# zgbkdlm/mfs

Hardware: AMD Instinct MI355X
Metric: filter time-steps/sec (higher is better)
Workload: dtype f64

## Files before the change

include/mfs_hip.h:

```cpp
#ifndef MFS_HIP_H
#define MFS_HIP_H

#include <stdint.h>

#ifdef __cplusplus
extern "C" {
#endif

#define MFS_ABI_VERSION 2

#define MFS_OK 0
#define MFS_EINVAL (-1)
#define MFS_EUNSUPPORTED (-2)
#define MFS_EHIP (-3)
#define MFS_ENOMEM (-4)
#define MFS_ERCCL (-5)

#define MFS_MODE_RAW 0
#define MFS_MODE_CENTRAL 1
#define MFS_MODE_SCALED 2
#define MFS_MODE_ODD_TAIL 0x100

#define MFS_TRANS_OPERATOR 0
#define MFS_TRANS_GAUSSIAN 1
// ... 47 lines not shown
int mfs_pool_trim(int device);
int mfs_pool_stats(int device, uint64_t* device_bytes, uint64_t* pinned_bytes, uint64_t* device_allocs,
                   uint64_t* pinned_allocs);
int mfs_event_create(void** event);
int mfs_event_destroy(void* event);
int mfs_event_record(void* event, void* stream);
int mfs_event_elapsed_ms(void* start, void* stop, float* ms);

int mfs_filter_1d(const mfs_model_1d* model, int mode, int N, int T, int B,
                  const double* m0, int m0_batched, const double* mean0, const double* scale0,
                  const double* ys, int stable,
                  double* out_moments, double* out_means, double* out_scales, double* out_nell,
                  int32_t* out_first_nan, int device, void* stream);

typedef struct mfs_plan_1d mfs_plan_1d;

int mfs_plan_1d_create(mfs_plan_1d** plan, const mfs_model_1d* model , int mode, int N,
                       int T, int B, int stable, int chunk, int device);
int mfs_plan_1d_run(mfs_plan_1d* plan, const double* d_m0, int m0_batched, const double* d_mean0,
                    const double* d_scale0, const double* d_ys, double* d_out_moments, double* d_out_means,
                    double* d_out_scales, double* d_out_nell, int32_t* d_out_first_nan, void* stream);
int mfs_plan_1d_destroy(mfs_plan_1d* plan);
int mfs_plan_1d_geometry(const mfs_plan_1d* plan, int* lanes_per_filter, int* filters_per_block, int* grid,
                         int* lds_bytes_per_block);
#define MFS_BUILD_DENSE 0
#define MFS_BUILD_FAST 1
#define MFS_BUILD_FAST_ONE_WAVE 2
#define MFS_BUILD_FAST_ONE_WAVE_SPEC 3
int mfs_plan_1d_kernel_build(const mfs_plan_1d* plan, int* build);
#define MFS_TRAITS_RUNTIME 0
#define MFS_TRAITS_CENTRAL_TANH_BERNOULLI 1
#define MFS_TRAITS_CENTRAL_IDENTITY_GAUSSIAN 2
int mfs_plan_1d_kernel_traits(const mfs_plan_1d* plan, int* traits);

int mfs_filter_1d_grad(const mfs_model_1d* model, const double* dcoef, const double* dlik, int n_par, int mode, int N,
                       int T, int B, const double* m0, int m0_batched, const double* mean0, const double* scale0,
                       const double* ys, double* out_nell, double* out_grad, int32_t* out_first_nan, int device,
                       void* stream);

int mfs_quadrature_1d(int N, int B, const double* ms, const double* mean, const double* scale, int stable,
                      double* out_weights, double* out_nodes, int device, void* stream);

int mfs_characteristic_1d(int N, int count, const double* ms, const double* mean, const double* scale, int nz,
                          const double* zs, double* out, int device, void* stream);

int mfs_elementary(int which, int n, const double* x, double* out, int device);

#define MFS_ND_TERMS 14
#define MFS_ND_TERMS_MAX 27
#define MFS_ND_ROWS 16
#define MFS_ND_ROWS_MAX 29
#define MFS_ND_TABLE_ROWS(n_terms) ((n_terms) > MFS_ND_TERMS ? MFS_ND_ROWS_MAX : MFS_ND_ROWS)
#define MFS_ND_MAX_EXTENT 6
#define MFS_ND_MAX_EXTENT_HI 7
#define MFS_ND_MAX_FACTORS 2
#define MFS_ND_TRANS_OPERATOR 0
#define MFS_ND_TRANS_GAUSSIAN 1
typedef struct mfs_model_nd {
    int32_t d;
    int32_t trans_kind;
    int32_t n_terms;
    int32_t extent;
    int32_t n_factors;
    int32_t ny;
    int32_t fac_kind[MFS_ND_MAX_FACTORS];
    int32_t fac_component[MFS_ND_MAX_FACTORS];
// ... 131 lines not shown
```

mfs_amd/_lib.py:

```python
import ctypes as C
import os

import numpy as np

_HERE = os.path.dirname(os.path.abspath(__file__))
LIB_PATH = os.path.join(_HERE, 'libmfs_hip.so')

MFS_OK = 0
MODE = {'raw': 0, 'central': 1, 'scaled': 2}
MODE_ODD_TAIL = 0x100
TRANS = {'operator': 0, 'gaussian': 1}
UMAP = {'x': 0, 'tanh': 1}
LIK = {'bernoulli_logistic': 0, 'poisson_softplus': 1, 'gaussian': 2, 'bearing_gaussian': 3}
MAX_N = 32
GRID_MAX_N = 8192
PF_MAX_PARTICLES = 1 << 20
PF_MAX_MIX = 8
RESAMPLE = {'stratified': 0, 'systematic': 1}
GF_METHOD = {'sigma_point': 0, 'ekf': 1}
GF_MAX_POINTS = 256

c_double_p = C.POINTER(C.c_double)
c_int32_p = C.POINTER(C.c_int32)

# ... 62 lines not shown
    ('mfs_version', _i, []),
    ('mfs_last_error', C.c_char_p, []),
    ('mfs_device_count', _i, [C.POINTER(C.c_int)]),
    ('mfs_set_device', _i, [_i]),
    ('mfs_device_synchronize', _i, []),
    ('mfs_device_name', _i, [_i, C.c_char_p, _i]),
    ('mfs_malloc', _i, [_vpp, _u64]),
    ('mfs_free', _i, [_vp]),
    ('mfs_memcpy_h2d', _i, [_vp, _vp, _u64, _vp]),
    ('mfs_memcpy_d2h', _i, [_vp, _vp, _u64, _vp]),
    ('mfs_memset', _i, [_vp, _i, _u64, _vp]),
    ('mfs_host_alloc', _i, [_vpp, _u64, _i]),
    ('mfs_host_free', _i, [_vp]),
    ('mfs_pool_trim', _i, [_i]),
    ('mfs_pool_stats', _i, [_i, C.POINTER(_u64), C.POINTER(_u64), C.POINTER(_u64), C.POINTER(_u64)]),
    ('mfs_stream_create', _i, [_vpp]),
    ('mfs_stream_destroy', _i, [_vp]),
    ('mfs_stream_synchronize', _i, [_vp]),
    ('mfs_event_create', _i, [_vpp]),
    ('mfs_event_destroy', _i, [_vp]),
    ('mfs_event_record', _i, [_vp, _vp]),
    ('mfs_event_elapsed_ms', _i, [_vp, _vp, C.POINTER(C.c_float)]),
    ('mfs_filter_1d', _i, [C.POINTER(MfsModel1d), _i, _i, _i, _i, _vp, _i, _vp, _vp, _vp, _i,
                           _vp, _vp, _vp, _vp, _vp, _i, _vp]),
    ('mfs_filter_1d_grad', _i, [C.POINTER(MfsModel1d), _vp, _vp, _i, _i, _i, _i, _i, _vp, _i, _vp, _vp, _vp, _vp, _vp, _vp,
                                _i, _vp]),
    ('mfs_plan_1d_create', _i, [_vpp, C.POINTER(MfsModel1d), _i, _i, _i, _i, _i, _i, _i]),
    ('mfs_plan_1d_run', _i, [_vp, _vp, _i, _vp, _vp, _vp, _vp, _vp, _vp, _vp, _vp, _vp]),
    ('mfs_plan_1d_destroy', _i, [_vp]),
    ('mfs_plan_1d_geometry', _i, [_vp, C.POINTER(C.c_int), C.POINTER(C.c_int), C.POINTER(C.c_int),
                                  C.POINTER(C.c_int)]),
    ('mfs_plan_1d_kernel_build', _i, [_vp, C.POINTER(C.c_int)]),
    ('mfs_plan_1d_kernel_traits', _i, [_vp, C.POINTER(C.c_int)]),
    ('mfs_quadrature_1d', _i, [_i, _i, _vp, _vp, _vp, _i, _vp, _vp, _i, _vp]),
    ('mfs_characteristic_1d', _i, [_i, _i, _vp, _vp, _vp, _i, _vp, _vp, _i, _vp]),
    ('mfs_filter_nd', _i, [C.POINTER(MfsModelNd), _i, _i, _i, _i, _i, _vp, _vp, _vp, _i, _vp, _vp, _vp, _i,
                           _vp, _vp, _vp, _vp, _vp, _i, _vp]),
    ('mfs_plan_nd_create', _i, [_vpp, C.POINTER(MfsModelNd), _i, _i, _i, _i, _i, _vp, _vp, _i, _i]),
    ('mfs_plan_nd_run', _i, [_vp, _vp, _i, _vp, _vp, _vp, _vp, _vp, _vp, _vp, _vp, _vp]),
    ('mfs_plan_nd_destroy', _i, [_vp]),
    ('mfs_plan_nd_geometry', _i, [_vp, C.POINTER(C.c_int), C.POINTER(C.c_int), C.POINTER(C.c_int)]),
    ('mfs_filter_nd3', _i, [C.POINTER(MfsModelNd3), _i, _i, _i, _i, _i, _vp, _vp, _vp, _i, _vp, _vp, _vp, _i,
                            _vp, _vp, _vp, _vp, _vp, _i, _vp]),
    ('mfs_plan_nd3_create', _i, [_vpp, C.POINTER(MfsModelNd3), _i, _i, _i, _i, _i, _vp, _vp, _i, _i]),
    ('mfs_plan_nd3_run', _i, [_vp, _vp, _i, _vp, _vp, _vp, _vp, _vp, _vp, _vp, _vp, _vp]),
    ('mfs_plan_nd3_destroy', _i, [_vp]),
    ('mfs_plan_nd3_geometry', _i, [_vp, C.POINTER(C.c_int), C.POINTER(C.c_int), C.POINTER(C.c_int)]),
    ('mfs_filter_nd3_joint', _i, [C.POINTER(MfsModelNd3), C.POINTER(MfsJointNd3), _i, _i, _i, _i, _i, _vp, _vp, _vp, _i, _vp,
                                  _vp, _vp, _i, _vp, _vp, _vp, _vp, _vp, _i, _vp]),
    ('mfs_plan_nd3_create_joint', _i, [_vpp, C.POINTER(MfsModelNd3), C.POINTER(MfsJointNd3), _i, _i, _i, _i, _i, _vp, _vp, _i,
                                       _i]),
    ('mfs_elementary', _i, [_i, _i, _vp, _vp, _i]),
    ('mfs_grid_filter_1d', _i, [_i, _i, _i, _i, _i, _vp, _vp, _vp, _i, _i, _vp, _i, _vp, _i, _vp,
                                _vp, _vp, _vp, _vp, _vp, _i, _vp]),
    ('mfs_grid_gemm_dev', _i, [_i, _i, _i, _vp, _vp, _vp, _vp]),
    ('mfs_particle_filter_1d', _i, [C.POINTER(MfsModel1d), _i, _i, _i, _i, _vp, _i, _vp, _vp, _vp, _vp, _i, _vp, _i, _vp,
                                    _vp, _vp, _vp, _vp, _vp, _vp, _i, _vp]),
    ('mfs_pf_draws', _i, [_u64, _i, _i, _i, _i, _vp, _vp, _i]),
    ('mfs_pf_last_split_ms', _i, [_vp]),
    ('mfs_gaussian_filter_1d', _i, [C.POINTER(MfsModel1d), _i, _i, _vp, _vp, _i, _i, _vp, _vp, _i, _vp, _vp, _vp, _vp, _vp,
                                    _i, _vp]),
    ('mfs_gaussian_filter_nd', _i, [C.POINTER(MfsModelNd), _i, _i, _vp, _vp, _i, _i, _vp, _vp, _i, _vp, _vp, _vp, _vp, _vp,
                                    _i, _vp]),
    ('mfs_comm_unique_id', _i, [_vp]),
    ('mfs_comm_init', _i, [_vpp, _vp, _i, _i, _i]),
    ('mfs_allgather_nell', _i, [_vp, _vp, _vp, _u64, _vp]),
# ... 137 lines not shown
```

mfs_amd/csrc/capi.hip:

```cpp
#include <hip/hip_runtime.h>

#include <cmath>
#include <cstdarg>
#include <cstdio>
#include <cstdlib>
#include <cstring>
#include <dlfcn.h>
#include <mutex>
#include <string>
#include <vector>

#include "filternd_kernel.hpp"
#include "filternd3_kernel.hpp"
#include "filter1d_grad.hpp"
#include "registry.hpp"
#include "staging.hpp"

namespace mfs {
KernelEntry g_table[MFS_MAX_N + 1][kSlots];
FastEntry g_fast[MFS_MAX_N + 1][4];

thread_local std::string g_err;

int fail(int code, const char* fmt, ...) {
// ... 46 lines not shown
    if (const char* e = getenv("MFS_LANES_PER_FILTER")) want = atoi(e);
    if ((stable != 0 || odd_tail != 0) && want != 0) dense = true;
    if (dense) {
        int gi = (N <= 16) ? 0 : (N <= 32) ? 1 : 2;
        if (want == 64) gi = 2;
        else if (want == 32 && N <= 32) gi = 1;
        else if (want == 16 && N <= 16) gi = 0;
        return gi;
    }
    int gi = mfs::default_group(N);
    if (want == 64) gi = 2;
    else if (want == 32 && N + 1 <= 32) gi = 1;
    else if (want == 16 && N + 1 <= 16) gi = 0;
    else if (want == 8 && N + 1 <= 8) gi = 3;
    return 3 + gi;
}

int check_run_pointers(int mode, const double* m0, const double* mean0, const double* scale0, const double* ys,
                       const double* out_nell, int T, int B) {
    if (!m0 || !out_nell || (T > 0 && B > 0 && !ys)) return fail(MFS_EINVAL, "m0 / ys / out_nell must not be NULL");
    if (mode != MFS_MODE_RAW && !mean0) return fail(MFS_EINVAL, "mean0 is required in central and scaled modes");
    if (mode == MFS_MODE_SCALED && !scale0) return fail(MFS_EINVAL, "scale0 is required in scaled mode");
    return MFS_OK;
}

}

struct mfs_plan_1d {
    mfs_model_1d model;
    int mode, N, T, B, stable, chunk, device, extra;
    int G, fpb, grid, lds_bytes, lds_doubles;
    mfs::Filter1dLaunch launch = nullptr;
    int launch_lds = 0, build = MFS_BUILD_DENSE, traits = MFS_TRAITS_RUNTIME;
    double* d_coef = nullptr;
    double* d_lik = nullptr;
    double* c_mom = nullptr;
    double* c_mean = nullptr;
    double* c_scale = nullptr;
    double* c_nell = nullptr;
    int32_t* c_first_nan = nullptr;
    double* c_lam = nullptr;
    hipStream_t own_stream = nullptr;
    hipGraph_t graph = nullptr;
    hipGraphExec_t exec = nullptr;
    const void* key[10] = {nullptr};
    int key_m0_batched = -1;
};

extern "C" {

int mfs_version(void) { return MFS_ABI_VERSION; }
const char* mfs_last_error(void) { return mfs::g_err.c_str(); }

int mfs_device_count(int* count) {
    if (!count) return fail(MFS_EINVAL, "count is NULL");
    HIP_TRY(hipGetDeviceCount(count));
    return MFS_OK;
}
int mfs_set_device(int device) { HIP_TRY(hipSetDevice(device)); return MFS_OK; }
int mfs_device_synchronize(void) { HIP_TRY(hipDeviceSynchronize()); return MFS_OK; }
int mfs_device_name(int device, char* buf, int buflen) {
    if (!buf || buflen <= 0) return fail(MFS_EINVAL, "bad buffer");
    hipDeviceProp_t p;
    HIP_TRY(hipGetDeviceProperties(&p, device));
    snprintf(buf, buflen, "%s (%s, %d CUs)", p.name, p.gcnArchName, p.multiProcessorCount);
    return MFS_OK;
// ... 47 lines not shown
    if (p->graph) hipGraphDestroy(p->graph);
    mfs::BlockPool<false>& pool = mfs::device_state(p->device).device;
    for (void* b : {(void*)p->d_coef, (void*)p->d_lik, (void*)p->c_mom, (void*)p->c_mean, (void*)p->c_scale,
                    (void*)p->c_nell, (void*)p->c_first_nan, (void*)p->c_lam})
        pool.release(b);
    if (p->own_stream) hipStreamDestroy(p->own_stream);
    delete p;
}

int mfs_plan_1d_destroy(mfs_plan_1d* p) {
    if (p) destroy_plan_1d(p, false);
    return MFS_OK;
}

static void resolve_launch(mfs_plan_1d* p, int slot, bool ext) {
    if (slot < 3) {
        p->launch = mfs::g_table[p->N][slot].filter; p->launch_lds = p->lds_bytes; p->build = MFS_BUILD_DENSE;
        return;
    }
    const mfs::FastEntry& fe = mfs::g_fast[p->N][slot - 3];
    int cus = 0;
    const bool one_wave = hipDeviceGetAttribute(&cus, hipDeviceAttributeMultiprocessorCount, p->device) == hipSuccess &&
                          p->grid <= 4 * cus;
    mfs::Filter1dFastLaunch spec = nullptr, wide = one_wave ? (ext ? fe.ext_wide : fe.wide) : nullptr;
    if (one_wave && !ext && ((p->model.degree + 4) & ~3) <= mfs::kSpecTop) {
        const int shape = mfs::spec_shape_index((p->model.trans_kind == MFS_TRANS_OPERATOR) ? p->model.n_terms : -1);
        const char* e = getenv("MFS_FAST_BUILD");
        if (shape >= 0 && !(e && strcmp(e, "generic") == 0)) spec = fe.spec[shape];
        const int ti = mfs::traits_index(p->mode, p->model.umap, p->model.lik_kind);
        const char* et = getenv("MFS_FAST_TRAITS");
        if (spec && ti != MFS_TRAITS_RUNTIME && !(et && strcmp(et, "runtime") == 0) && fe.spec_traits[shape][ti - 1]) {
            spec = fe.spec_traits[shape][ti - 1];
            p->traits = ti;
        }
    }
    p->launch = spec ? spec : wide ? wide : ext ? fe.ext : fe.filter;
    p->launch_lds = p->lds_doubles;
    p->build = spec ? MFS_BUILD_FAST_ONE_WAVE_SPEC : wide ? MFS_BUILD_FAST_ONE_WAVE : MFS_BUILD_FAST;
}

int mfs_plan_1d_create(mfs_plan_1d** plan, const mfs_model_1d* model, int mode, int N, int T, int B, int stable,
                       int chunk, int device) {
    if (!plan) return fail(MFS_EINVAL, "plan is NULL");
    *plan = nullptr;
    if (int rc = check_model(model, mode)) return rc;
    if (N < 2 || N > MFS_MAX_N) return fail(MFS_EUNSUPPORTED, "N = %d outside [2, %d]", N, MFS_MAX_N);
    if (T < 0 || B < 0) return fail(MFS_EINVAL, "negative T or B");
    if (chunk < 0) return fail(MFS_EINVAL, "negative chunk");
    const int extra = (mode & MFS_MODE_ODD_TAIL) ? 1 : 0;
    mode &= 0xff;
    if (extra && chunk != 0 && chunk < T) return fail(MFS_EUNSUPPORTED, "an odd moment count runs in one launch (chunk = 0)");
    const int slot = pick_slot(N, stable, extra);
    const mfs::KernelEntry& ke = mfs::g_table[N][slot];
    if (!ke.quad) return fail(MFS_EUNSUPPORTED, "no kernel compiled for N = %d", N);
    HIP_TRY(hipSetDevice(device));

    mfs_plan_1d* p = new mfs_plan_1d();
    p->model = *model;
    p->mode = mode; p->N = N; p->T = T; p->B = B; p->stable = stable; p->device = device; p->extra = extra;
    p->chunk = (chunk == 0 || chunk > T) ? T : chunk;
    p->G = ke.lanes_per_filter;
    p->fpb = ke.waves_per_block * (64 / p->G);
    p->grid = (B + p->fpb - 1) / p->fpb;
    p->lds_doubles = ke.lds_doubles_per_filter;
    if (slot >= 3) p->lds_doubles += ((model->degree + 4) & ~3) * 10;
    const bool ext = slot >= 3 && (stable != 0 || extra != 0);
// ... 15 lines not shown
    alloc((void**)&p->c_mean, (size_t)B * 8);
    alloc((void**)&p->c_scale, (size_t)B * 8);
    alloc((void**)&p->c_nell, (size_t)B * 8);
    alloc((void**)&p->c_first_nan, (size_t)B * 4);
    if (p->chunk < T && slot >= 3) alloc((void**)&p->c_lam, (size_t)B * 2 * p->G * 8);
    if (e == hipSuccess) e = hipMemcpy(p->d_coef, model->coef, ncoef * 8, hipMemcpyHostToDevice);
    if (e == hipSuccess) e = hipMemcpy(p->d_lik, model->lik, nlik * 8, hipMemcpyHostToDevice);
    if (e != hipSuccess) {
        destroy_plan_1d(p, true);
        return fail(e == hipErrorOutOfMemory ? MFS_ENOMEM : MFS_EHIP, "plan setup failed: %s", hipGetErrorString(e));
    }
    p->model.coef = p->d_coef;
    p->model.lik = p->d_lik;
    *plan = p;
    return MFS_OK;
}

int mfs_plan_1d_geometry(const mfs_plan_1d* p, int* lanes_per_filter, int* filters_per_block, int* grid,
                         int* lds_bytes_per_block) {
    if (!p) return fail(MFS_EINVAL, "plan is NULL");
    if (lanes_per_filter) *lanes_per_filter = p->G;
    if (filters_per_block) *filters_per_block = p->fpb;
    if (grid) *grid = p->grid;
    if (lds_bytes_per_block) *lds_bytes_per_block = p->lds_bytes;
    return MFS_OK;
}

int mfs_plan_1d_kernel_build(const mfs_plan_1d* p, int* build) {
    if (!p || !build) return fail(MFS_EINVAL, "plan or build is NULL");
    *build = p->build;
    return MFS_OK;
}

int mfs_plan_1d_kernel_traits(const mfs_plan_1d* p, int* traits) {
    if (!p || !traits) return fail(MFS_EINVAL, "plan or traits is NULL");
    *traits = p->traits;
    return MFS_OK;
}

static int enqueue_chunks(mfs_plan_1d* p, const mfs::Filter1dArgs& base, hipStream_t s) {
    mfs::Filter1dArgs a = base;
    int t0 = 0;
    do {
        a.t_begin = t0;
        a.t_end = (t0 + p->chunk < p->T) ? t0 + p->chunk : p->T;
        hipError_t e = p->launch(a, p->grid, p->launch_lds, s);
        if (e != hipSuccess) return fail(MFS_EHIP, "kernel launch failed: %s", hipGetErrorString(e));
    } while ((t0 += p->chunk) < p->T);
    return MFS_OK;
}

static mfs::Filter1dArgs plan_args(const mfs_plan_1d* p, const double* d_m0, int m0_batched, const double* d_mean0,
                                    const double* d_scale0, const double* d_ys, double* d_out_moments,
                                    double* d_out_means, double* d_out_scales, double* d_out_nell,
                                    int32_t* d_out_first_nan) {
    mfs::Filter1dArgs a;
    memset(&a, 0, sizeof(a));
    a.mode = p->mode; a.T = p->T; a.B = p->B; a.stable = p->stable; a.extra = p->extra;
    a.trans_kind = p->model.trans_kind; a.umap = p->model.umap; a.n_terms = p->model.n_terms;
    a.degree = p->model.degree; a.n_rows = p->model.n_rows; a.coef_batched = p->model.coef_batched;
    a.lik_kind = p->model.lik_kind; a.n_lik = p->model.n_lik; a.lik_batched = p->model.lik_batched;
    a.mean_x_coef = p->model.mean_x_coef; a.coef = p->model.coef; a.lik = p->model.lik;
    a.m0 = d_m0; a.m0_batched = m0_batched; a.mean0 = d_mean0; a.scale0 = d_scale0; a.ys = d_ys;
    a.c_mom = p->c_mom; a.c_mean = p->c_mean; a.c_scale = p->c_scale; a.c_nell = p->c_nell;
    a.c_first_nan = p->c_first_nan;
    a.c_lam = p->c_lam;
    if (const char* e = getenv("MFS_PREDICT_RULE")) a.recompute_rule = (strcmp(e, "recompute") == 0);
    a.out_mom = d_out_moments; a.out_mean = (p->mode != MFS_MODE_RAW) ? d_out_means : nullptr;
    a.out_scale = (p->mode == MFS_MODE_SCALED) ? d_out_scales : nullptr;
    a.out_nell = d_out_nell; a.out_first_nan = d_out_first_nan;
    return a;
}

int mfs_plan_1d_run(mfs_plan_1d* p, const double* d_m0, int m0_batched, const double* d_mean0,
                    const double* d_scale0, const double* d_ys, double* d_out_moments, double* d_out_means,
                    double* d_out_scales, double* d_out_nell, int32_t* d_out_first_nan, void* stream) {
    if (!p) return fail(MFS_EINVAL, "plan is NULL");
    if (int rc = check_run_pointers(p->mode, d_m0, d_mean0, d_scale0, d_ys, d_out_nell, p->T, 1)) return rc;
    if (p->B == 0) return MFS_OK;
// ... 46 lines not shown
                  void* stream) {
    const int extra = (mode & MFS_MODE_ODD_TAIL) ? 1 : 0, full_mode = mode;
    mode &= 0xff;
    if (int rc = check_run_pointers(mode, m0, mean0, scale0, ys, out_nell, T, B)) return rc;
    const size_t M2 = 2 * (size_t)N + extra, nb = m0_batched ? B : 1;
    const int nchunks = extra ? 1 : host_chunks(device, T, B, M2, out_moments != nullptr);
    const int chunk = (nchunks > 1) ? (T + nchunks - 1) / nchunks : 0;
    mfs_plan_1d* p = nullptr;
    if (int rc = mfs_plan_1d_create(&p, model, full_mode, N, T, B, stable, chunk, device)) return rc;
    struct PlanGuard { mfs_plan_1d* p; ~PlanGuard() { destroy_plan_1d(p, true); } } guard{p};
    if (B == 0) return MFS_OK;

    mfs::Staging st(device, stream, true);
    double *d_m0 = nullptr, *d_mean0 = nullptr, *d_scale0 = nullptr, *d_ys = nullptr, *d_mom = nullptr,
           *d_means = nullptr, *d_scales = nullptr, *d_nell = nullptr;
    int32_t* d_fn = nullptr;
    st.alloc(&d_m0, nb * M2 * 8);
    st.alloc(&d_mean0, nb * 8);
    st.alloc(&d_scale0, nb * 8);
    st.alloc(&d_ys, (size_t)B * T * 8);
    if (out_moments) st.alloc(&d_mom, (size_t)B * T * M2 * 8);
    if (out_means && mode != MFS_MODE_RAW) st.alloc(&d_means, (size_t)B * T * 8);
    if (out_scales && mode == MFS_MODE_SCALED) st.alloc(&d_scales, (size_t)B * T * 8);
    st.alloc(&d_nell, (size_t)B * 8);
    st.alloc(&d_fn, (size_t)B * 4);
    st.h2d(d_m0, m0, nb * M2 * 8);
    if (mean0) st.h2d(d_mean0, mean0, nb * 8);
    if (scale0) st.h2d(d_scale0, scale0, nb * 8);
    st.h2d(d_ys, ys, (size_t)B * T * 8);

    mfs::Filter1dArgs a = plan_args(p, d_m0, m0_batched, d_mean0, d_scale0, d_ys, d_mom, d_means, d_scales, d_nell, d_fn);
    const int rc = mfs::run_streaming_out(st, T, B, nchunks, M2, out_moments, d_mom, [&](int t0, int t1) {
        a.t_begin = t0; a.t_end = t1;
        const hipError_t e = p->launch(a, p->grid, p->launch_lds, st.s);
        return (e == hipSuccess) ? MFS_OK : fail(MFS_EHIP, "kernel launch failed: %s", hipGetErrorString(e));
    });
    if (rc == MFS_OK) {
        st.d2h(out_means, d_means, (size_t)B * T * 8);
        st.d2h(out_scales, d_scales, (size_t)B * T * 8);
        st.d2h(out_nell, d_nell, (size_t)B * 8);
        st.d2h(out_first_nan, d_fn, (size_t)B * 4);
    }
    return st.finish("mfs_filter_1d", rc);
}

int mfs_filter_1d_grad(const mfs_model_1d* model, const double* dcoef, const double* dlik, int n_par, int mode, int N,
                       int T, int B, const double* m0, int m0_batched, const double* mean0, const double* scale0,
                       const double* ys, double* out_nell, double* out_grad, int32_t* out_first_nan, int device,
                       void* stream) {
    if (int rc = check_model(model, mode)) return rc;
    if (mode & MFS_MODE_ODD_TAIL) return fail(MFS_EUNSUPPORTED, "the gradient entry point takes 2N moments");
    if (n_par < 1 || n_par > mfs::kGradMaxP) return fail(MFS_EUNSUPPORTED, "n_par = %d outside [1, %d]", n_par, mfs::kGradMaxP);
    if (N < 2 || N > mfs::kGradMaxN)
        return fail(MFS_EUNSUPPORTED, "N = %d outside [2, %d] for the gradient kernel", N, mfs::kGradMaxN);
    if (T < 0 || B < 0) return fail(MFS_EINVAL, "negative T or B");
    if (!dcoef || !dlik || !out_grad) return fail(MFS_EINVAL, "NULL buffer");
    if (int rc = check_run_pointers(mode, m0, mean0, scale0, ys, out_nell, T, B)) return rc;
    if (B == 0) return MFS_OK;
    mfs::Filter1dGradLaunch launch = mfs::g_grad_table[N][n_par];
    if (!launch) return fail(MFS_EUNSUPPORTED, "no gradient kernel compiled for N = %d, n_par = %d", N, n_par);
    HIP_TRY(hipSetDevice(device));
    mfs::Staging st(device, stream, true);
    const size_t J1 = (size_t)model->degree + 1, ncoef = (size_t)model->n_rows * J1;
    const size_t nbc = model->coef_batched ? B : 1, nbl = model->lik_batched ? B : 1, nb = m0_batched ? B : 1, M2 = 2 * (size_t)N;
    double *d_coef = nullptr, *d_dcoef = nullptr, *d_lik = nullptr, *d_dlik = nullptr, *d_m0 = nullptr, *d_mean0 = nullptr,
           *d_scale0 = nullptr, *d_ys = nullptr, *d_nell = nullptr, *d_grad = nullptr;
    int32_t* d_fn = nullptr;
// ... 1049 lines not shown
```

mfs_amd/csrc/registry.hpp:

```cpp
#pragma once
#include <hip/hip_runtime.h>

#include "../../include/mfs_hip.h"

namespace mfs {

struct Filter1dArgs;
struct Quad1dArgs;
struct Cf1dArgs;
struct Filter1dGradArgs;
struct FilterNdArgs;
struct FilterNd3Args;
struct FilterNd3Joint;

using Filter1dLaunch = hipError_t (*)(const Filter1dArgs&, int grid, int lds_bytes, hipStream_t);
using Quad1dLaunch = hipError_t (*)(const Quad1dArgs&, int grid, int lds_bytes, hipStream_t);
using Filter1dFastLaunch = hipError_t (*)(const Filter1dArgs&, int grid, int lds_doubles_per_filter, hipStream_t);
using Cf1dLaunch = hipError_t (*)(const Cf1dArgs&, int grid, int lds, hipStream_t);

struct KernelEntry {
    Filter1dLaunch filter;
    Quad1dLaunch quad;
    int lds_doubles_per_filter;
    int waves_per_block;
    int lanes_per_filter;
};

constexpr int kSlots = 7;
extern KernelEntry g_table[MFS_MAX_N + 1][kSlots];

constexpr int group_lanes(const int gi) { return (gi == 3) ? 8 : 16 << gi; }
constexpr int default_group(const int N) { return (N + 1 <= 8) ? 3 : (N + 1 <= 16) ? 0 : (N + 1 <= 32) ? 1 : 2; }

constexpr int kSpecShapes = 4;
constexpr int spec_shape_index(const int spec) { return (spec == -1) ? 0 : (spec == 2) ? 1 : (spec == 4) ? 2 : (spec == 6) ? 3 : -1; }

constexpr int kTraitSets = 2;
constexpr int traits_index(const int mode, const int umap, const int lik_kind) {
    return (mode != MFS_MODE_CENTRAL) ? MFS_TRAITS_RUNTIME
         : (umap == MFS_U_TANH && lik_kind == MFS_LIK_BERNOULLI_LOGISTIC) ? MFS_TRAITS_CENTRAL_TANH_BERNOULLI
         : (umap == MFS_U_IDENTITY && lik_kind == MFS_LIK_GAUSSIAN) ? MFS_TRAITS_CENTRAL_IDENTITY_GAUSSIAN
         : MFS_TRAITS_RUNTIME;
}

struct FastEntry {
    Filter1dFastLaunch filter;
    Filter1dFastLaunch wide;
    Filter1dFastLaunch ext, ext_wide;
    Filter1dFastLaunch spec[kSpecShapes];
    Filter1dFastLaunch spec_traits[kSpecShapes][kTraitSets];
    Quad1dLaunch quad_ext;
    Cf1dLaunch cf;
    int ext_shift;
    int quad_ext_lds;
};
extern FastEntry g_fast[MFS_MAX_N + 1][4];

using Filter1dGradLaunch = hipError_t (*)(const Filter1dGradArgs&, int n_filters, hipStream_t);
constexpr int kGradMaxN = 16, kGradMaxP = 4;
extern Filter1dGradLaunch g_grad_table[kGradMaxN + 1][kGradMaxP + 1];

using FilterNdLaunch = hipError_t (*)(const FilterNdArgs&, int grid, hipStream_t);
struct NdEntry { FilterNdLaunch launch, launch_gauss, launch_hi, launch_joint; int S, Z, lds_bytes, carry_doubles; };
constexpr int kNdMaxN = 7;
extern NdEntry g_nd_table[kNdMaxN + 1];
hipError_t launch_elementary(int which, int n, const double* d_x, double* d_out, hipStream_t s);

using FilterNd3Launch = hipError_t (*)(const FilterNd3Args&, int grid, hipStream_t);
using FilterNd3JointLaunch = hipError_t (*)(const FilterNd3Args&, const FilterNd3Joint&, int grid, hipStream_t);
struct Nd3Entry { FilterNd3Launch launch, launch_gauss; int S, Z, lds_bytes; FilterNd3JointLaunch joint, joint_gauss; };
extern Nd3Entry g_nd3_table[MFS_ND3_MAX_N + 1];

constexpr int kGridTile = 64;
constexpr int kGridBK = 16;

inline int grid_pad(const int v) { return (v + kGridTile - 1) / kGridTile * kGridTile; }

struct GridUpdateArgs {
    int n, T, B, t;
    int ldp;
    int lik_kind, n_lik, lik_batched;
    const double* xs;
    const double* w;
    const double* lik;
    const double* ys;
    double* P;
    double* out_pdfs;
    double* out_means;
    double* out_vars;
// ... 94 lines not shown
```

Measured before the change: 453.7 million.

## Add partner-wave 1D filter kernel splitting predict/update from moment recompute

Adds a specialised kernel for orders 14-15 in central mode with fixed traits. Each workgroup pairs four main waves, which run prediction, quadrature and the likelihood update, with four partner waves that rebuild posterior moments, accumulate the log-likelihood and write outputs. The two sets of waves exchange data through LDS with double-buffered flags and s_barrier, so the moment work overlaps the next step's main-wave work. It also adds a per-workgroup SIMD placement counter using atomics, which costs a little per launch, and needs more LDS and threads per block. The plan selects this kernel by default when eligible and falls back to the one-wave kernel for recompute-rule runs.

```diff
diff --git a/include/mfs_hip.h b/include/mfs_hip.h
--- a/include/mfs_hip.h
+++ b/include/mfs_hip.h
@@ -103,6 +103,8 @@
 #define MFS_TRAITS_CENTRAL_TANH_BERNOULLI 1
 #define MFS_TRAITS_CENTRAL_IDENTITY_GAUSSIAN 2
 int mfs_plan_1d_kernel_traits(const mfs_plan_1d* plan, int* traits);
+int mfs_plan_1d_kernel_partner(const mfs_plan_1d* plan, int* partner);
+int mfs_partner_placement(uint64_t* workgroups, uint64_t* mismatches);
 
 int mfs_filter_1d_grad(const mfs_model_1d* model, const double* dcoef, const double* dlik, int n_par, int mode, int N,
                        int T, int B, const double* m0, int m0_batched, const double* mean0, const double* scale0,
diff --git a/mfs_amd/_lib.py b/mfs_amd/_lib.py
--- a/mfs_amd/_lib.py
+++ b/mfs_amd/_lib.py
@@ -118,6 +118,8 @@
                                   C.POINTER(C.c_int)]),
     ('mfs_plan_1d_kernel_build', _i, [_vp, C.POINTER(C.c_int)]),
     ('mfs_plan_1d_kernel_traits', _i, [_vp, C.POINTER(C.c_int)]),
+    ('mfs_plan_1d_kernel_partner', _i, [_vp, C.POINTER(C.c_int)]),
+    ('mfs_partner_placement', _i, [C.POINTER(_u64), C.POINTER(_u64)]),
     ('mfs_quadrature_1d', _i, [_i, _i, _vp, _vp, _vp, _i, _vp, _vp, _i, _vp]),
     ('mfs_characteristic_1d', _i, [_i, _i, _vp, _vp, _vp, _i, _vp, _vp, _i, _vp]),
     ('mfs_filter_nd', _i, [C.POINTER(MfsModelNd), _i, _i, _i, _i, _i, _vp, _vp, _vp, _i, _vp, _vp, _vp, _i,
diff --git a/mfs_amd/csrc/capi.hip b/mfs_amd/csrc/capi.hip
--- a/mfs_amd/csrc/capi.hip
+++ b/mfs_amd/csrc/capi.hip
@@ -102,6 +102,8 @@
     int G, fpb, grid, lds_bytes, lds_doubles;
     mfs::Filter1dLaunch launch = nullptr;
     int launch_lds = 0, build = MFS_BUILD_DENSE, traits = MFS_TRAITS_RUNTIME;
+    int partner = 0, one_wave_grid = 0;
+    mfs::Filter1dFastLaunch one_wave_launch = nullptr;
     double* d_coef = nullptr;
     double* d_lik = nullptr;
     double* c_mom = nullptr;
@@ -215,6 +217,16 @@
         if (spec && ti != MFS_TRAITS_RUNTIME && !(et && strcmp(et, "runtime") == 0) && fe.spec_traits[shape][ti - 1]) {
             spec = fe.spec_traits[shape][ti - 1];
             p->traits = ti;
+            const char* ep = getenv("MFS_FAST_PARTNER");
+            const int lds = mfs::partner_lds_bytes(p->lds_doubles, fe.partner_doubles);
+            if (fe.partner[shape][ti - 1] && !(ep && strcmp(ep, "0") == 0) && lds <= mfs::kPartnerLdsMax) {
+                p->partner = 1;
+                p->one_wave_launch = spec; p->one_wave_grid = p->grid;
+                spec = fe.partner[shape][ti - 1];
+                p->fpb = mfs::kPartnerFilters;
+                p->grid = (p->B + p->fpb - 1) / p->fpb;
+                p->lds_bytes = lds;
+            }
         }
     }
     p->launch = spec ? spec : wide ? wide : ext ? fe.ext : fe.filter;
@@ -296,6 +308,31 @@
     return MFS_OK;
 }
 
+int mfs_plan_1d_kernel_partner(const mfs_plan_1d* p, int* partner) {
+    if (!p || !partner) return fail(MFS_EINVAL, "plan or partner is NULL");
+    *partner = p->partner;
+    return MFS_OK;
+}
+
+int mfs_partner_placement(uint64_t* workgroups, uint64_t* mismatches) {
+    if (!workgroups || !mismatches) return fail(MFS_EINVAL, "workgroups or mismatches is NULL");
+    uint64_t sum[2] = {0, 0};
+    for (int N = 0; N <= MFS_MAX_N; ++N)
+        for (int gi = 0; gi < 4; ++gi)
+            if (mfs::PartnerPlacementRead read = mfs::g_fast[N][gi].partner_placement) {
+                unsigned long long c[2] = {0, 0};
+                HIP_TRY(read(c));
+                sum[0] += c[0]; sum[1] += c[1];
+            }
+    *workgroups = sum[0]; *mismatches = sum[1];
+    return MFS_OK;
+}
+
+static hipError_t plan_launch(const mfs_plan_1d* p, const mfs::Filter1dArgs& a, hipStream_t s) {
+    if (p->partner && a.recompute_rule) return p->one_wave_launch(a, p->one_wave_grid, p->launch_lds, s);
+    return p->launch(a, p->grid, p->launch_lds, s);
+}
+
 int mfs_plan_1d_kernel_traits(const mfs_plan_1d* p, int* traits) {
     if (!p || !traits) return fail(MFS_EINVAL, "plan or traits is NULL");
     *traits = p->traits;
@@ -308,7 +345,7 @@
     do {
         a.t_begin = t0;
         a.t_end = (t0 + p->chunk < p->T) ? t0 + p->chunk : p->T;
-        hipError_t e = p->launch(a, p->grid, p->launch_lds, s);
+        hipError_t e = plan_launch(p, a, s);
         if (e != hipSuccess) return fail(MFS_EHIP, "kernel launch failed: %s", hipGetErrorString(e));
     } while ((t0 += p->chunk) < p->T);
     return MFS_OK;
@@ -421,7 +458,7 @@
     mfs::Filter1dArgs a = plan_args(p, d_m0, m0_batched, d_mean0, d_scale0, d_ys, d_mom, d_means, d_scales, d_nell, d_fn);
     const int rc = mfs::run_streaming_out(st, T, B, nchunks, M2, out_moments, d_mom, [&](int t0, int t1) {
         a.t_begin = t0; a.t_end = t1;
-        const hipError_t e = p->launch(a, p->grid, p->launch_lds, st.s);
+        const hipError_t e = plan_launch(p, a, st.s);
         return (e == hipSuccess) ? MFS_OK : fail(MFS_EHIP, "kernel launch failed: %s", hipGetErrorString(e));
     });
     if (rc == MFS_OK) {
diff --git a/mfs_amd/csrc/filter1d_partner.hpp b/mfs_amd/csrc/filter1d_partner.hpp
--- /dev/null
+++ b/mfs_amd/csrc/filter1d_partner.hpp
@@ -0,0 +1,361 @@
+#pragma once
+#include "filter1d_fast.hpp"
+
+namespace mfs {
+
+#ifndef MFS_PARTNER_AB_LOGPY
+#define MFS_PARTNER_AB_LOGPY 0
+#endif
+
+constexpr int kPartnerMainWaves = 4;
+constexpr int kPartnerThreads = 2 * kPartnerMainWaves * 64;
+
+static __device__ unsigned long long g_partner_placement[2];
+
+template <int N, int G>
+struct PartnerTile {
+    using L = FastTile<N, G>;
+    static constexpr int oMom = 0;
+    static constexpr int oTab = L::M2;
+    static constexpr int oXch = oTab + G * L::TLD;
+    static constexpr int oFlag = oXch + 2 * 4 * G;
+    static constexpr int kDoubles = oFlag + 2;
+    static_assert((kDoubles & 1) == 0, "tiles stay 16-byte aligned");
+};
+constexpr int kPartnerFlagDead = 1, kPartnerFlagPivot = 2;
+
+__device__ __forceinline__ void partner_barrier() {
+    asm volatile("s_waitcnt lgkmcnt(0)\n\ts_barrier" ::: "memory");
+}
+
+template <int N, int G, int SPEC, class TR>
+__global__ __launch_bounds__(kPartnerThreads, 2) void filter1d_partner_kernel(const Filter1dArgs a, const int lds_doubles) {
+    static_assert(G == 16 && N + 1 <= G, "orders with 16 lanes per filter");
+    static_assert(TR::fixed && TR::mode == MFS_MODE_CENTRAL, "fixed step traits, central mode");
+    static_assert(SPEC == -1 || SPEC == 6, "table shapes with a fixed-traits build");
+    using L = FastTile<N, G>;
+    using P = PartnerTile<N, G>;
+    constexpr int M2 = L::M2, TLD = L::TLD;
+    constexpr int FPW = 64 / G, FPB = kPartnerMainWaves * FPW;
+    constexpr bool kLogMain = (MFS_PARTNER_AB_LOGPY != 0);
+    extern __shared__ __attribute__((aligned(16))) double smem[];
+    const int lane = threadIdx.x & 63, wave = __builtin_amdgcn_readfirstlane((int)(threadIdx.x >> 6));
+    const bool is_main = wave < kPartnerMainWaves;
+    const int grp = lane / G, l = lane - grp * G;
+    const int slot = (wave & (kPartnerMainWaves - 1)) * FPW + grp;
+    const int b = blockIdx.x * FPB + slot;
+    const bool has = b < a.B;
+    double* S = smem + (size_t)slot * lds_doubles;
+    double* PS = smem + (size_t)FPB * lds_doubles + (size_t)slot * P::kDoubles;
+    double* xch = PS + P::oXch;
+    int* flags = reinterpret_cast<int*>(PS + P::oFlag);
+    const double qnan = __builtin_nan("");
+    const bool node = (l < N);
+
+    {
+        int* simd = reinterpret_cast<int*>(smem + (size_t)FPB * lds_doubles + P::oXch);
+        unsigned hw;
+        asm volatile("s_getreg_b32 %0, hwreg(HW_REG_HW_ID)" : "=s"(hw));
+        if (lane == 0) simd[wave] = (int)((hw >> 4) & 3u);
+        __syncthreads();
+        if (threadIdx.x == 0) {
+            bool same = true;
+            for (int w = 0; w < kPartnerMainWaves; ++w) same &= simd[w] == simd[w + kPartnerMainWaves];
+            atomicAdd(&g_partner_placement[0], 1ull);
+            if (!same) atomicAdd(&g_partner_placement[1], 1ull);
+        }
+        __syncthreads();
+    }
+
+    if (is_main) {
+        double* mom = S + L::oMom;
+        double* TAB = S + L::oTab;
+        const double* coef = S + L::oCoef;
+        const double* lp = S + L::oLik;
+        double* lfac = S + L::oLfac;
+        const int J1 = a.degree + 1;
+        if (has) {
+            const double* src = a.coef + (a.coef_batched ? (size_t)b * a.n_rows * J1 : 0);
+            for (int e = l; e < ((a.degree + 4) & ~3) * kCoefRows; e += G) {
+                const int j = e / kCoefRows, r = e - j * kCoefRows;
+                int sr = r;
+                if (a.trans_kind == MFS_TRANS_OPERATOR) sr = (r == MFS_MAX_TERMS) ? a.n_terms : (r < a.n_terms) ? r : a.n_rows;
+                S[L::oCoef + e] = (sr < a.n_rows && j < J1) ? src[sr * J1 + j] : 0.0;
+            }
+            const double* ls = a.lik + (a.lik_batched ? (size_t)b * a.n_lik : 0);
+            for (int e = l; e < MFS_MAX_LIK; e += G) S[L::oLik + e] = (e < a.n_lik) ? ls[e] : 0.0;
+            if (TR::lik == MFS_LIK_POISSON_SOFTPLUS)
+                for (int e = l; e <= kLfacMax; e += G) lfac[e] = log_factorial((double)e);
+        }
+        double mean = 0.0, scale = 1.0, nell = 0.0;
+        int first_nan = -1;
+        double gA = qnan, gW = 0.0;
+        bool have_atoms = false;
+        if (has) {
+            if (a.t_begin == 0) {
+                const double* src = a.m0 + (a.m0_batched ? (size_t)b * M2 : 0);
+                for (int n = l; n < M2; n += G) mom[n] = src[n];
+                mean = a.mean0[a.m0_batched ? b : 0];
+            } else {
+                if (!a.c_lam) for (int n = l; n < M2; n += G) mom[n] = a.c_mom[(size_t)b * M2 + n];
+                mean = a.c_mean[b];
+                scale = a.c_scale[b];
+                if constexpr (kLogMain) nell = a.c_nell[b];
+                first_nan = a.c_first_nan[b];
+                if (a.c_lam) {
+                    gA = a.c_lam[((size_t)b * 2 + 0) * G + l];
+                    gW = a.c_lam[((size_t)b * 2 + 1) * G + l];
+                    have_atoms = true;
+                }
+            }
+        }
+        wave_sync();
+        constexpr int SR = (SPEC > 0) ? SPEC + 1 : 2;
+        constexpr int kVarReg = (SPEC > 0) ? SPEC : -1;
+        double tabr[kSpecTop][SR];
+        LikRegs lpr;
+#pragma unroll
+        for (int q = 0; q < kSpecTop; ++q)
+#pragma unroll
+            for (int r = 0; r < SR; ++r) tabr[q][r] = coef[q * kCoefRows + ((r == kVarReg) ? MFS_MAX_TERMS : r)];
+#pragma unroll
+        for (int e = 0; e < MFS_MAX_LIK; ++e) lpr.v[e] = lp[e];
+        const bool st_mean = has && a.out_mean && (l == 0);
+        size_t o_mean = (size_t)b * a.T + a.t_begin;
+        const double* yrow = a.ys + (size_t)b * a.T;
+        bool dead = !has || (first_nan >= 0);
+        asm volatile("" : "+v"(mean), "+v"(scale), "+v"(nell), "+v"(gA), "+v"(gW), "+v"(first_nan));
+        double ywin = 0.0;
+        constexpr int kSlUpdate = kSlEigLoop;
+        constexpr int trans_kind = (SPEC > 0) ? MFS_TRANS_OPERATOR : MFS_TRANS_GAUSSIAN;
+
+        for (int t = a.t_begin; t < a.t_end; ++t) {
+            constexpr int YW = 16;
+            const int tw = (t - a.t_begin) & (YW - 1);
+            if (tw == 0) {
+                const double ld = (has && t + (l & (YW - 1)) < a.t_end) ? yrow[t + (l & (YW - 1))] : 0.0;
+                asm volatile("v_mov_b64 %0, %1" : "=v"(ywin) : "v"(ld));
+            }
+            const double y = __shfl(ywin, tw, YW);
+            double* xs = xch + (t & 1) * 4 * G;
+            double nell_next = nell;
+            if (!dead) {
+                int bad = 0;
+                double gB = qnan;
+                auto predict = [&](const auto atoms_ok) __attribute__((always_inline)) {
+                    double x, w;
+                    double lam_io = gA;
+                    if constexpr (decltype(atoms_ok)::value) {
+                        x = node ? fma(scale, lam_io, mean) : mean;
+                        w = node ? gW : 0.0;
+                    } else {
+                        quadrature_fast<N, G, false>(mom, l, grp, mean, scale, x, w, lam_io, false, false, gW, S, a.stable);
+                    }
+                    gB = lam_io;
+                    const double u = (TR::umap == MFS_U_TANH) ? fast_tanh(x) : x;
+                    double c = 0.0, inv_sc = 1.0;
+                    double rows[MFS_MAX_TERMS + 1];
+                    {
+                        double live[SR];
+                        horner_regs<kSpecTop, SR>(tabr, u, live);
+#pragma unroll
+                        for (int r = 0; r <= MFS_MAX_TERMS; ++r) rows[r] = 0.0;
+#pragma unroll
+                        for (int r = 0; r < SR; ++r) rows[(r == kVarReg) ? MFS_MAX_TERMS : r] = live[r];
+                    }
+                    double mu, var;
+                    if (trans_kind == MFS_TRANS_OPERATOR) {
+                        mu = x + rows[0];
+                        var = rows[MFS_MAX_TERMS];
+                    } else {
+                        mu = fma(a.mean_x_coef, x, rows[0]);
+                        var = rows[1];
+                    }
+                    mean = gsum<G>(w * mu);
+                    c = mean;
+                    double* row = TAB + l * TLD;
+                    if (trans_kind == MFS_TRANS_OPERATOR) {
+                        operator_moments<(SPEC > 0) ? SPEC : 2, M2>(rows, x - c, w, inv_sc, node, row);
+                    } else {
+                        const double ms = (mu - c) * inv_sc, vs = var * inv_sc * inv_sc;
+                        double f2 = w, f1 = w * ms, vn = vs;
+                        row[0] = f2;
+                        row[1] = f1;
+#pragma unroll
+                        for (int n = 2; n < M2; ++n) {
+                            const double f = fma(ms, f1, vn * f2);
+                            row[n] = f;
+                            vn += vs;
+                            f2 = f1;
+                            f1 = f;
+                        }
+                    }
+                    wave_sync();
+                    {
+                        const int n0 = l, n1 = l + G;
+                        const bool has0 = n0 < M2, has1 = n1 < M2;
+                        const double* t0 = TAB + (has0 ? n0 : 0);
+                        const double* t1 = TAB + (has1 ? n1 : 0);
+                        double c0[N], c1[N];
+#pragma unroll
+                        for (int i = 0; i < N; ++i) { c0[i] = t0[i * TLD]; c1[i] = t1[i * TLD]; }
+                        __builtin_amdgcn_sched_barrier(0);
+                        double s0[3] = {0.0, 0.0, 0.0}, s1[3] = {0.0, 0.0, 0.0};
+#pragma unroll
+                        for (int i = 0; i < N; ++i) { s0[i % 3] += c0[i]; s1[i % 3] += c1[i]; }
+                        const double acc0 = (s0[0] + s0[1]) + s0[2], acc1 = (s1[0] + s1[1]) + s1[2];
+                        if (has0) { mom[n0] = acc0; bad |= !finite(acc0); }
+                        if (has1) { mom[n1] = acc1; bad |= !finite(acc1); }
+                    }
+                    wave_sync();
+                };
+                if (have_atoms) predict(std::true_type{});
+                else predict(std::false_type{});
+                {
+                    double x, w;
+                    double lam_io = gB;
+                    quadrature_fast<N, G, false, kSlUpdate>(mom, l, grp, mean, scale, x, w, lam_io, true, false, gW, S, a.stable);
+                    double c = 0.0, inv_sc = 1.0, py = 1.0, ipy = 1.0;
+                    const double wl = node ? w * likelihood_sel<true>(TR::lik, lpr, lp, lfac, y, x) : 0.0;
+                    py = gsum<G>(wl);
+                    ipy = rcp_nr(py);
+                    mean = gsum<G>(wl * x) * ipy;
+                    c = mean;
+                    double dx;
+                    {
+#pragma clang fp contract(off)
+                        dx = (x - c) * inv_sc;
+                    }
+                    {
+                        const double last = bcast<G, N - 1>(dx);
+                        gA = node ? dx : last;
+                        gW = wl * ipy;
+                        have_atoms = true;
+                    }
+                    if constexpr (kLogMain) {
+                        nell_next = nell - fast_log(py);
+                        bad |= (int)!finite(nell_next);
+                    }
+                    bad |= (int)(!finite(mean) || !finite(scale));
+                    xs[0 * G + l] = dx;
+                    xs[1 * G + l] = wl;
+                    xs[2 * G + l] = ipy;
+                    xs[3 * G + l] = py;
+                    flags[2 + (t & 1)] = gany<G>(bad != 0, grp) ? 1 : 0;
+                }
+            }
+            partner_barrier();
+            const int fl = flags[(t + 1) & 1];
+            if (dead || fl != 0) {
+                dead = true;
+                mean = qnan; scale = qnan;
+                if constexpr (kLogMain) nell = qnan;
+            } else {
+                if constexpr (kLogMain) nell = nell_next;
+            }
+            if (st_mean) a.out_mean[o_mean] = mean;
+            o_mean += 1;
+        }
+        if (has) {
+            if (a.t_end >= a.T) {
+                if constexpr (kLogMain) { if (l == 0) a.out_nell[b] = nell; }
+            } else {
+                if (a.c_lam) { a.c_lam[((size_t)b * 2 + 0) * G + l] = gA; a.c_lam[((size_t)b * 2 + 1) * G + l] = gW; }
+                if (l == 0) {
+                    a.c_mean[b] = mean; a.c_scale[b] = scale;
+                    if constexpr (kLogMain) a.c_nell[b] = nell;
+                }
+            }
+        }
+    } else {
+        double* pmom = PS + P::oMom;
+        double* PTAB = PS + P::oTab;
+        double nell = 0.0;
+        int first_nan = -1;
+        bool pivot_prev = false;
+        double xd, wd, lamd = qnan;
+        if (has && a.t_begin != 0) {
+            for (int n = l; n < M2; n += G) pmom[n] = a.c_mom[(size_t)b * M2 + n];
+            if constexpr (!kLogMain) nell = a.c_nell[b];
+            first_nan = a.c_first_nan[b];
+        }
+        wave_sync();
+        bool dead = !has || (first_nan >= 0);
+        if (!dead && a.t_begin != 0)
+            pivot_prev = quadrature_fast<N, G, false>(pmom, l, grp, 0.0, 1.0, xd, wd, lamd, false, true, 0.0, PS, 0);
+        flags[(a.t_begin + 1) & 1] = (dead ? kPartnerFlagDead : 0) | (pivot_prev ? kPartnerFlagPivot : 0);
+        const bool st_m0 = has && a.out_mom && l < M2, st_m1 = has && a.out_mom && l + G < M2;
+        size_t o_mom = ((size_t)b * a.T + a.t_begin) * M2 + l;
+
+        for (int t = a.t_begin; t < a.t_end; ++t) {
+            partner_barrier();
+            const double* xs = xch + (t & 1) * 4 * G;
+            double out0 = qnan, out1 = qnan;
+            if (!dead && !pivot_prev) {
+                int bad = flags[2 + (t & 1)];
+                const double dx = xs[0 * G + l], wl = xs[1 * G + l], ipy = xs[2 * G + l], py = xs[3 * G + l];
+                double* row = PTAB + l * TLD;
+                {
+                    const double dx2 = dx * dx, dx4 = dx2 * dx2;
+                    double pw[4] = {wl, wl * dx, wl * dx2, wl * dx2 * dx};
+#pragma unroll
+                    for (int n = 0; n < M2; ++n) {
+                        row[n] = pw[n & 3];
+                        pw[n & 3] *= dx4;
+                    }
+                }
+                if constexpr (!kLogMain) nell -= fast_log(py);
+                wave_sync();
+                {
+                    const int n0 = l, n1 = l + G;
+                    const bool has0 = n0 < M2, has1 = n1 < M2;
+                    const double* t0 = PTAB + (has0 ? n0 : 0);
+                    const double* t1 = PTAB + (has1 ? n1 : 0);
+                    double c0[N], c1[N];
+#pragma unroll
+                    for (int i = 0; i < N; ++i) { c0[i] = t0[i * TLD]; c1[i] = t1[i * TLD]; }
+                    __builtin_amdgcn_sched_barrier(0);
+                    double s0[3] = {0.0, 0.0, 0.0}, s1[3] = {0.0, 0.0, 0.0};
+#pragma unroll
+                    for (int i = 0; i < N; ++i) { s0[i % 3] += c0[i]; s1[i % 3] += c1[i]; }
+                    double acc0 = (s0[0] + s0[1]) + s0[2], acc1 = (s1[0] + s1[1]) + s1[2];
+                    acc0 *= ipy; acc1 *= ipy;
+                    if (has0) { pmom[n0] = acc0; bad |= !finite(acc0); }
+                    if (has1) { pmom[n1] = acc1; bad |= !finite(acc1); }
+                    out0 = acc0; out1 = acc1;
+                }
+                wave_sync();
+                if constexpr (!kLogMain) bad |= (int)!finite(nell);
+                if (gany<G>(bad != 0, grp)) { dead = true; first_nan = t; }
+                pivot_prev = quadrature_fast<N, G, false>(pmom, l, grp, 0.0, 1.0, xd, wd, lamd, false, true, 0.0, PS, 0);
+            } else {
+                if (!dead) first_nan = t;
+                dead = true;
+                pivot_prev = false;
+                for (int n = l; n < M2; n += G) pmom[n] = qnan;
+                nell = qnan;
+                wave_sync();
+            }
+            flags[t & 1] = (dead ? kPartnerFlagDead : 0) | (pivot_prev ? kPartnerFlagPivot : 0);
+            if (st_m0) a.out_mom[o_mom] = out0;
+            if (st_m1) a.out_mom[o_mom + G] = out1;
+            o_mom += M2;
+        }
+        if (has) {
+            if (a.t_end >= a.T) {
+                if (l == 0) {
+                    if constexpr (!kLogMain) a.out_nell[b] = nell;
+                    if (a.out_first_nan) a.out_first_nan[b] = first_nan;
+                }
+            } else {
+                for (int n = l; n < M2; n += G) a.c_mom[(size_t)b * M2 + n] = pmom[n];
+                if (l == 0) {
+                    if constexpr (!kLogMain) a.c_nell[b] = nell;
+                    a.c_first_nan[b] = first_nan;
+                }
+            }
+        }
+    }
+}
+
+}
diff --git a/mfs_amd/csrc/filter1d_partner_inst.hip b/mfs_amd/csrc/filter1d_partner_inst.hip
--- /dev/null
+++ b/mfs_amd/csrc/filter1d_partner_inst.hip
@@ -0,0 +1,46 @@
+#include "filter1d_partner.hpp"
+#include "launch_util.hpp"
+#include "registry.hpp"
+
+#ifndef MFS_SPEC_N
+#error "compile with -DMFS_SPEC_N=14..15"
+#endif
+
+namespace mfs {
+
+template <int N, int G, int SPEC, class TR>
+hipError_t launch_filter_partner(const Filter1dArgs& a, int grid, int lds_doubles, hipStream_t s) {
+    const int lds_bytes = partner_lds_bytes(lds_doubles, PartnerTile<N, G>::kDoubles);
+    if (lds_bytes > kPartnerLdsMax) return hipErrorInvalidValue;
+    if (hipError_t e = ensure_dynamic_lds<&filter1d_partner_kernel<N, G, SPEC, TR>>(kPartnerLdsMax); e != hipSuccess) return e;
+    hipLaunchKernelGGL((filter1d_partner_kernel<N, G, SPEC, TR>), dim3(grid), dim3(kPartnerThreads), lds_bytes, s, a, lds_doubles);
+    return hipGetLastError();
+}
+
+static hipError_t read_partner_placement(unsigned long long* counts) {
+    return hipMemcpyFromSymbol(counts, HIP_SYMBOL(g_partner_placement), 2 * sizeof(*counts));
+}
+
+namespace {
+struct PartnerRegistrar {
+    PartnerRegistrar() {
+        constexpr int N = MFS_SPEC_N;
+        static_assert(N >= 14 && N <= 15, "orders with 16 lanes per filter and a one-wave build");
+        constexpr int gi = default_group(N), G = group_lanes(gi);
+        static_assert(G == 16, "lanes per filter");
+        static_assert(kPartnerFilters == kPartnerMainWaves * (64 / G), "filters per workgroup");
+        using TanhBernoulli = StepTraits<MFS_MODE_CENTRAL, MFS_U_TANH, MFS_LIK_BERNOULLI_LOGISTIC>;
+        using IdentityGaussian = StepTraits<MFS_MODE_CENTRAL, MFS_U_IDENTITY, MFS_LIK_GAUSSIAN>;
+        constexpr int tb = MFS_TRAITS_CENTRAL_TANH_BERNOULLI - 1, ig = MFS_TRAITS_CENTRAL_IDENTITY_GAUSSIAN - 1;
+        FastEntry& fe = g_fast[N][gi];
+        fe.partner[spec_shape_index(6)][tb] = &launch_filter_partner<N, G, 6, TanhBernoulli>;
+        fe.partner[spec_shape_index(-1)][tb] = &launch_filter_partner<N, G, -1, TanhBernoulli>;
+        fe.partner[spec_shape_index(-1)][ig] = &launch_filter_partner<N, G, -1, IdentityGaussian>;
+        fe.partner_doubles = PartnerTile<N, G>::kDoubles;
+        fe.partner_placement = &read_partner_placement;
+    }
+};
+PartnerRegistrar partner_registrar_instance;
+}
+
+}
diff --git a/mfs_amd/csrc/registry.hpp b/mfs_amd/csrc/registry.hpp
--- a/mfs_amd/csrc/registry.hpp
+++ b/mfs_amd/csrc/registry.hpp
@@ -43,18 +43,29 @@
          : MFS_TRAITS_RUNTIME;
 }
 
+using PartnerPlacementRead = hipError_t (*)(unsigned long long counts[2]);
+
 struct FastEntry {
     Filter1dFastLaunch filter;
     Filter1dFastLaunch wide;
     Filter1dFastLaunch ext, ext_wide;
     Filter1dFastLaunch spec[kSpecShapes];
     Filter1dFastLaunch spec_traits[kSpecShapes][kTraitSets];
+    Filter1dFastLaunch partner[kSpecShapes][kTraitSets];
+    int partner_doubles;
+    PartnerPlacementRead partner_placement;
     Quad1dLaunch quad_ext;
     Cf1dLaunch cf;
     int ext_shift;
     int quad_ext_lds;
 };
 extern FastEntry g_fast[MFS_MAX_N + 1][4];
+
+constexpr int kPartnerFilters = 16;
+constexpr int kPartnerLdsMax = 160 * 1024;
+constexpr int partner_lds_bytes(const int lds_doubles_per_filter, const int partner_doubles) {
+    return kPartnerFilters * (lds_doubles_per_filter + partner_doubles) * 8;
+}
 
 using Filter1dGradLaunch = hipError_t (*)(const Filter1dGradArgs&, int n_filters, hipStream_t);
 constexpr int kGradMaxN = 16, kGradMaxP = 4;
```

Result: faster. 536.9 million (median of 6 runs) (+18.3%).
